# pvachon/tsl-sdr

Hardware: AMD Instinct MI355X
Metric: input IQ MSamp/s x channels demodulated (higher is better)
Workload: dtype int16

## Files before the change

tsl-sdr_amd/csrc/mfm_kernel.h:

```cpp
#pragma once

#include <stdint.h>

#define MFM_WAVE 64
#define MFM_CG 8
#define MFM_TG 2
#define MFM_NW 8
#define MFM_NT (MFM_NW * MFM_WAVE)

struct mfm_chan_info {
    uint64_t rot_base;
    uint32_t mu;
    uint32_t lam;
    uint32_t lam_magic;
    uint32_t pad0;
    uint32_t out_row;
    uint32_t rot_class;
};

#define MFM_RC_GENERAL 0u
#define MFM_RC_QUARTER 1u
#define MFM_RC_FLIP 2u
#define MFM_RC_IDENT 3u

// ... 127 lines not shown
    uint32_t stream_taps;
    uint32_t row_bytes;
    uint32_t split_rows;
    uint32_t kq_used;
    uint32_t nh;
    uint32_t kperm[4];
    uint32_t ng;
    uint32_t rb;
    uint32_t nstage_p;
    uint32_t shift;
    uint32_t tp_off;
    uint32_t *tail_dst;
    unsigned long long *cyc;
    unsigned long long *cyc_clear;
    uint32_t cyc_tag, pad2;
    const uint32_t *afrag;
    const int32_t *krow;
    const struct mfm_chan_info *info;
    const void *rot;
    const float2 *lut;
    int16_t *pcm;
    uint32_t *iq_dbg;
    const uint32_t *head;
    uint32_t head_n, pad3;
};
```

tsl-sdr_amd/csrc/mfm_kernel_v3.hip:

```cpp
#include <hip/hip_runtime.h>

#include <type_traits>

#include "mfm_kernel.h"
#include "mfm_numerics.h"

#include "mfm_v3_device.h"

#define MFM3_MF(d, a, b, c) "v_mfma_i32_16x16x64_i8 %[" #d "], %[" #a "], %[" #b "], " c "\n\t"
#define MFM3_RD(d, o) "ds_read_b128 %[" #d "], %[lb] offset:%[" #o "]\n\t"
#define MFM3_LA(d, a, b) "v_lshl_add_u32 %[" #d "], %[" #a "], 8, %[" #b "]\n\t"
#define MFM3_SH0(d, a) "v_lshrrev_b32_sdwa %[" #d "], 14, %[" #a "] dst_sel:WORD_0 dst_unused:UNUSED_PAD src0_sel:DWORD src1_sel:DWORD\n\t"
#define MFM3_SH1(d, a) "v_lshrrev_b32_sdwa %[" #d "], 14, %[" #a "] dst_sel:WORD_1 dst_unused:UNUSED_PRESERVE src0_sel:DWORD src1_sel:DWORD\n\t"

template <bool HAS_PREV, bool HAS_NEXT, int LO, int O2, int O3, int N0, int N1, bool REUSE = false>
static __device__ __forceinline__ void mfm3_group_d96(uint32_t lb, uint32_t ka, const mfm_v4i &al0, const mfm_v4i &al1,
                                                      const mfm_v4i &al2, const mfm_v4i &al3, const mfm_v4i &ah1,
                                                      const mfm_v4i &ah2, mfm_v4i &b0h, mfm_v4i &b0l, mfm_v4i &b1h,
                                                      mfm_v4i &b1l, mfm_v4i &b2h, mfm_v4i &b2l, const mfm_v4i (&accP)[3],
                                                      mfm_v4i (&acc)[3], uint32_t (&tP)[4])
{
    mfm_v4i hh, md, ll;
    uint32_t t0 = 0, t1 = 0, t2 = 0, t3 = 0;
    if (HAS_PREV) {
// ... 260 lines not shown
    static constexpr bool padded = DFIX == 25;
    static constexpr uint32_t row_bytes = padded ? 64u : 2u * D;
    static constexpr bool chunk_rows = !padded && (2u * D) % 64u != 0u;
    static constexpr uint32_t rows = padded ? MFM_V3_LEAD + MFM_V3_OT + 5u
                                            : MFM_V3_LEAD + MFM_V3_OT + (64u * 4u - 1u) / (2u * D);
    static constexpr uint32_t cpo = D / 8u, per = 4u * cpo;
    static constexpr uint32_t nchunks16 = (rows * 2u * D + 15u) / 16u;
    static constexpr uint32_t pitch_a = (nchunks16 + per - 1u) / per + 1u, pitch_b = 16u + 1u + (cpo * 3u + 12u) / per + 1u;
    static constexpr uint32_t pitch = pitch_a > pitch_b ? pitch_a : pitch_b;
    static constexpr uint32_t plane_t = ((per + 3u) * pitch * 16u + 63u) & ~63u;
    static constexpr uint32_t rs = padded ? 96u : mfm3_row_stride(D), sp = MFM3_SP;
    static constexpr uint32_t plane_pitch = chunk_rows ? plane_t : 4u * sp, buf_pitch = 2u * plane_pitch;
    static constexpr uint32_t ofs(uint32_t g, uint32_t kq)
    {
        if (chunk_rows) {
            const uint32_t x = cpo * g + 4u * kq;
            return ((x % per) * pitch + 1u + x / per) * 16u;
        }
        const uint32_t c = (64u * kq) / row_bytes, w = (64u * kq) % row_bytes;
        return ((g + c) & 3u) * sp + (1u + ((g + c) >> 2)) * rs + w;
    }
};

template <int KQ, bool DBG_IQ, int NCH, int AHM, int DFIX, int IN8, uint32_t RC = MFM_RC_GENERAL>
__global__ __launch_bounds__(MFM3_NT, 4) void mfm_channel_kernel_v3(const mfm_launch_v3 L)
{
    extern __shared__ __attribute__((aligned(16))) uint8_t smem[];

    const uint32_t tid = threadIdx.x;
    const uint32_t lane = tid & 63u;
    const uint32_t wave = __builtin_amdgcn_readfirstlane(tid >> 6);
    const uint32_t kg = lane >> 4, n = lane & 15u;
    using G = mfm3_geo<DFIX>;
    constexpr bool PADDED = DFIX != 0 && G::padded;
    constexpr uint32_t NCHS = PADDED ? 4u : (uint32_t)NCH;
    const uint32_t D = DFIX ? (uint32_t)DFIX : L.decim, row_bytes = PADDED ? 64u : 2u * D;
    const uint32_t rs = DFIX ? G::rs : L.rs;
    const uint32_t sp_pitch = DFIX ? G::sp : L.sp_pitch;
    const uint32_t plane_pitch = DFIX ? G::plane_pitch : L.plane_pitch, buf_pitch = DFIX ? G::buf_pitch : L.buf_pitch;
    const bool chunk_rows = DFIX ? G::chunk_rows : L.layout == 1u;
    const uint32_t t_per = DFIX ? G::per : L.t_per, t_pitch = DFIX ? G::pitch : L.t_pitch;
    const uint32_t ah_mask = AHM >= 0 ? (uint32_t)AHM : (uint32_t)__builtin_amdgcn_readfirstlane(L.ah_mask);
    const uint32_t lut_addr = (uint32_t)(uintptr_t)(smem + L.lut_off) | (MFM3_LUT_MODE == 2 ? 1u : 0u);
    const bool pcm_sys = L.pcm_scope != 0u;

    static_assert(MFM3_NT == 512, "one table dword per thread");
    const uint32_t lut_v = reinterpret_cast<const uint32_t *>(L.lut)[tid];
#if !MFM3_PROLOGUE
    reinterpret_cast<uint32_t *>(smem + L.lut_off)[MFM3_LUT_SLOT(tid)] = lut_v;
#endif

    uint32_t *sta_s = reinterpret_cast<uint32_t *>(smem + L.sta_off);
    uint32_t *sta2_s = sta_s + NCHS * MFM3_NT + 768u;
    uint16_t *sta16_s = reinterpret_cast<uint16_t *>(sta_s);
    if constexpr (PADDED) {
        constexpr int C = IN8 ? 8 : 4;
        const int delta = ((int)L.hist - (int)(MFM_V3_LEAD * 25u)) & (C - 1);
#pragma unroll
        for (int k = 0; k < C; k++) {
            const int i = C * (int)tid + k - delta;
            uint32_t off = 64u;
            if (i >= 0 && i < (int)(G::rows * 25u)) {
                const uint32_t row = (uint32_t)i / 25u, col = ((uint32_t)i % 25u) * 2u;
                off = (row & 3u) * sp_pitch + (row >> 2) * rs + col;
            }
            sta16_s[tid * 8u + (uint32_t)k] = (uint16_t)off;
        }
    }
#pragma unroll
    for (int j = 0; j < NCH && !PADDED; j++) {
        const uint32_t p8 = (tid + (uint32_t)j * MFM3_NT) * (IN8 ? 16u : 8u);
        if (chunk_rows) {
            const uint32_t sc = p8 >> 4, r = sc % t_per, c = sc / t_per;
            sta_s[j * MFM3_NT + tid] = (r * t_pitch + c) * 16u + (p8 & 15u);
            sta2_s[j * MFM3_NT + tid] = (r < 3u && c >= 1u) ? ((r + t_per) * t_pitch + c - 1u) * 16u + (p8 & 15u) : 0xffffffffu;
        } else {
            const uint32_t row = p8 / row_bytes, colb = p8 % row_bytes;
            sta_s[j * MFM3_NT + tid] = (row & 3u) * sp_pitch + (row >> 2) * rs + colb;
        }
    }

    uint32_t ofs[4][KQ], ofs_w[KQ];
#pragma unroll
    for (int kq = 0; kq < KQ; kq++) {
        const uint32_t c = DFIX ? (64u * kq) / row_bytes : L.cross[kq], w = DFIX ? (64u * kq) % row_bytes : L.within[kq];
        static_assert(!PADDED || (KQ == 6 && NCH == 1), "decimation 25: six rows per window, one staging chunk per thread");
#pragma unroll
        for (int g = 0; g < 4; g++) {
            ofs[g][kq] = ((g + c) & 3u) * sp_pitch + (1u + ((g + c) >> 2)) * rs + w;
        }
        ofs_w[kq] = ((3u + c) & 3u) * sp_pitch + ((3u + c) >> 2) * rs + w;
        if (chunk_rows) {
            const uint32_t cpo = t_per >> 2;
#pragma unroll
            for (int g = 0; g < 4; g++) {
                const uint32_t x = cpo * (uint32_t)g + 4u * (uint32_t)kq;
                ofs[g][kq] = ((x % t_per) * t_pitch + 1u + x / t_per) * 16u;
            }
            const uint32_t xw = cpo * 3u + 4u * (uint32_t)kq;
            ofs_w[kq] = ((xw % t_per) * t_pitch + xw / t_per) * 16u;
        }
    }
    const uint32_t lb0 = chunk_rows ? 16u * n + 16u * t_pitch * kg : n * rs + 16u * kg;

    auto stage_index = [&](uint32_t tile, int j) -> int {
        const uint32_t q = tid + (uint32_t)j * MFM3_NT;
        int gs = (int)(tile * MFM_V3_OT * D + L.hist) - (int)(MFM_V3_LEAD * D) + (IN8 ? 8 : 4) * (int)(q < L.nstage4 ? q : 0u);
        if constexpr (PADDED) {
            gs -= ((int)L.hist - (int)(MFM_V3_LEAD * 25u)) & ((IN8 ? 8 : 4) - 1);
        }
        gs = gs < 0 ? 0 : gs;
        return gs > (int)L.x_last4 ? (int)L.x_last4 : gs;
    };
    auto stage_load = [&](uint32_t tile, int j) -> uint4 {
        const int gs = stage_index(tile, j);
#if MFM3_NONTEMPORAL & 1
        const mfm_v4i ld = __builtin_nontemporal_load(
            reinterpret_cast<const mfm_v4i *>(reinterpret_cast<const uint8_t *>(L.x) + ((uint32_t)gs << (IN8 ? 1 : 2))));
        return make_uint4((uint32_t)ld[0], (uint32_t)ld[1], (uint32_t)ld[2], (uint32_t)ld[3]);
#else
        return *reinterpret_cast<const uint4 *>(reinterpret_cast<const uint8_t *>(L.x) + ((uint32_t)gs << (IN8 ? 1 : 2)));
#endif
    };
    auto stage_store = [&](uint32_t buf, int j, const uint4 &v) {
        if constexpr (PADDED) {
            if (tid < L.nstage4) {
                const uint4 o = *reinterpret_cast<const uint4 *>(sta16_s + tid * 8u);
                uint8_t *img = smem + buf * buf_pitch;
                const uint32_t vv[4] = { v.x, v.y, v.z, v.w }, oo[4] = { o.x, o.y, o.z, o.w };
                if (IN8) {
                    const uint32_t m = L.in8_xor;
#pragma unroll
                    for (int k = 0; k < 4; k++) {
                        const uint32_t w = vv[k] ^ m;
                        *reinterpret_cast<uint16_t *>(img + (oo[k] & 0xffffu)) = (uint16_t)w;
                        *reinterpret_cast<uint16_t *>(img + (oo[k] >> 16)) = (uint16_t)(w >> 16);
                    }
                } else {
#pragma unroll
                    for (int k = 0; k < 4; k++) {
                        const uint32_t off = (k & 1) ? oo[k >> 1] >> 16 : oo[k >> 1] & 0xffffu;
                        const uint32_t hi = __builtin_amdgcn_perm(vv[k], vv[k], 0x0c0c0301u);
                        const uint32_t lo = __builtin_amdgcn_perm(vv[k], vv[k], 0x0c0c0200u) ^ 0x8080u;
                        *reinterpret_cast<uint16_t *>(img + off) = (uint16_t)hi;
                        *reinterpret_cast<uint16_t *>(img + off + plane_pitch) = (uint16_t)lo;
                    }
                }
            }
            (void)j;
            return;
        }
        if (IN8) {
            if (tid + (uint32_t)j * MFM3_NT < L.nstage4) {
                const uint32_t m = L.in8_xor;
                const uint4 w = make_uint4(v.x ^ m, v.y ^ m, v.z ^ m, v.w ^ m);
                *reinterpret_cast<uint4 *>(smem + buf * buf_pitch + sta_s[j * MFM3_NT + tid]) = w;
                if (chunk_rows) {
                    const uint32_t a2 = sta2_s[j * MFM3_NT + tid];
                    if (a2 != 0xffffffffu) {
                        *reinterpret_cast<uint4 *>(smem + buf * buf_pitch + a2) = w;
                    }
                }
            }
        } else if (tid + (uint32_t)j * MFM3_NT < L.nstage4) {
            uint2 hi, lo;
            hi.x = __builtin_amdgcn_perm(v.y, v.x, 0x07050301u);
            hi.y = __builtin_amdgcn_perm(v.w, v.z, 0x07050301u);
            lo.x = __builtin_amdgcn_perm(v.y, v.x, 0x06040200u) ^ 0x80808080u;
            lo.y = __builtin_amdgcn_perm(v.w, v.z, 0x06040200u) ^ 0x80808080u;
            uint8_t *base = smem + buf * buf_pitch + sta_s[j * MFM3_NT + tid];
            *reinterpret_cast<uint2 *>(base) = hi;
            *reinterpret_cast<uint2 *>(base + plane_pitch) = lo;
            if (chunk_rows) {
                const uint32_t a2 = sta2_s[j * MFM3_NT + tid];
                if (a2 != 0xffffffffu) {
                    uint8_t *b2 = smem + buf * buf_pitch + a2;
                    *reinterpret_cast<uint2 *>(b2) = hi;
                    *reinterpret_cast<uint2 *>(b2 + plane_pitch) = lo;
                }
            }
        }
    };

    if (blockIdx.x == 0) {
        for (uint32_t i = tid; i < L.tail_n; i += MFM3_NT) {
            if (IN8) {
                reinterpret_cast<uint16_t *>(L.tail_dst)[i] = reinterpret_cast<const uint16_t *>(L.x)[L.tail_src + i];
            } else {
                L.tail_dst[i] = L.x[L.tail_src + i];
            }
        }
    }

    uint32_t item = blockIdx.x, chunk, slice;
    if (!mfm3_decode_item(L, item, &chunk, &slice)) {
        return;
    }
    const uint32_t stamp_t0 = mfm3_stamp_lo(L.cyc ? __builtin_amdgcn_s_memtime() : 0ull), stamp_r0 = mfm3_stamp_lo(L.cyc ? __builtin_amdgcn_s_memrealtime() : 0ull);
    uint32_t tile = (uint32_t)(((uint64_t)chunk * L.ntiles) / L.nchunks);
    uint32_t tend = (uint32_t)(((uint64_t)(chunk + 1u) * L.ntiles) / L.nchunks);
    mfm_v4i a_h[KQ], a_l[KQ];
    mfm_v4i *krow_s = reinterpret_cast<mfm_v4i *>(smem + L.sta_off + NCHS * MFM3_NT * 4u) + wave * 4u + kg;
    uint32_t slice_loaded = 0xffffffffu;
    {
        uint4 v[NCH];
#pragma unroll
        for (int j = 0; j < NCH; j++) {
            v[j] = stage_load(tile, j);
        }
#if MFM3_PROLOGUE
        const uint32_t rb0 = slice * 8u + wave;
        mfm_v4i krow0 = { 0, 0, 0, 0 };
        if (rb0 < L.nrb) {
            const mfm_v4i *ap = reinterpret_cast<const mfm_v4i *>(L.afrag) + (size_t)rb0 * KQ * 2 * 64 + mfm3_opaque(lane);
#pragma unroll
            for (int kq = 0; kq < KQ; kq++) {
                a_h[kq] = ap[(kq * 2 + 0) * 64];
                a_l[kq] = ap[(kq * 2 + 1) * 64];
            }
            krow0 = *reinterpret_cast<const mfm_v4i *>(L.krow + (size_t)rb0 * 16 + 4 * mfm3_opaque(kg));
        }
        reinterpret_cast<uint32_t *>(smem + L.lut_off)[MFM3_LUT_SLOT(tid)] = lut_v;
#endif
        if constexpr (IN8 == 0) {
            if (L.head_n != 0u && tile == 0u) {
#pragma unroll
                for (int j = 0; j < NCH; j++) {
                    const uint32_t gs = (uint32_t)stage_index(0u, j);
                    uint32_t w[4] = { v[j].x, v[j].y, v[j].z, v[j].w };
#pragma unroll
                    for (int k = 0; k < 4; k++) {
                        if (gs + (uint32_t)k < L.head_n) {
                            w[k] = L.head[gs + (uint32_t)k];
                        }
                    }
                    v[j] = make_uint4(w[0], w[1], w[2], w[3]);
                }
            }
        }
#pragma unroll
        for (int j = 0; j < NCH; j++) {
            stage_store(0, j, v[j]);
        }
#if MFM3_PROLOGUE
        if (rb0 < L.nrb) {
            asm volatile("s_waitcnt vmcnt(0)" ::: "memory");
            if (n == 0) {
                *krow_s = krow0;
            }
#pragma unroll
            for (int kq = 0; kq < KQ; kq++) {
                asm volatile("" : "+v"(a_h[kq]), "+v"(a_l[kq]));
            }
            slice_loaded = slice;
        }
#endif
    }
    __syncthreads();

    const int prio_matrix = wave >= 4 ? 1 : 0;
    uint2 *fold_s = reinterpret_cast<uint2 *>(smem + L.sta_off + NCHS * MFM3_NT * 4u + 512u) + (wave * 4u + kg) * 2u;
    uint32_t *xq_s = reinterpret_cast<uint32_t *>(smem + L.sta_off + NCHS * MFM3_NT * 4u + 1024u) + (wave * 4u + kg) * 16u;
    uint32_t cur = 0;
    bool first_of_chunk = true;

    uint32_t kb8[2] = { 0, 0 };
    uint32_t voff[2] = { 0, 0 };
    uint32_t hist[2] = { 0, 0 };
    bool ch_ok[2] = { false, false };
    bool w_exact = false;

    auto advance = [&](uint32_t &it, uint32_t &ch, uint32_t &sl, uint32_t &ti, uint32_t &te, bool &first) -> bool {
        ti += 1u;
        first = false;
        if (ti >= te) {
            it += gridDim.x;
            const bool v = mfm3_decode_item(L, it, &ch, &sl);
            ti = (uint32_t)(((uint64_t)ch * L.ntiles) / L.nchunks);
            te = (uint32_t)(((uint64_t)(ch + 1u) * L.ntiles) / L.nchunks);
            first = true;
            return v;
        }
        return true;
    };
    constexpr bool EARLY = IN8 != 0 || MFM3_EARLY16;
    uint4 pre[NCH];
    if (EARLY) {
        uint32_t a_item = item, a_chunk = chunk, a_slice = slice, a_tile = tile, a_tend = tend;
        bool a_first = false;
        const bool a_valid = advance(a_item, a_chunk, a_slice, a_tile, a_tend, a_first);
#pragma unroll
        for (int j = 0; j < NCH; j++) {
            pre[j] = stage_load(a_valid ? a_tile : tile, j);
        }
    }

    while (true) {
        uint32_t n_item = item, n_chunk = chunk, n_slice = slice, n_tile = tile, n_tend = tend;
        bool n_first = false;
        const bool n_valid = advance(n_item, n_chunk, n_slice, n_tile, n_tend, n_first);
        if (!EARLY) {
#pragma unroll
            for (int j = 0; j < NCH; j++) {
                pre[j] = stage_load(n_valid ? n_tile : tile, j);
            }
            __builtin_amdgcn_sched_barrier(MFM3_SCHED_ALL_BUT_VMEM);
        }

        if (prio_matrix) {
            __builtin_amdgcn_s_setprio(1);
        } else {
            __builtin_amdgcn_s_setprio(0);
        }
        const uint32_t rb = slice * 8u + wave;
        const bool rb_valid = rb < L.nrb;
        const uint32_t lb = lb0 + cur * buf_pitch;
        const uint8_t *img = smem;
        const uint32_t first_out = tile * MFM_V3_OT;

        uint32_t f[4][2];
        uint4 rva[2][MFM3_ROT4 ? 1 : 2];
        if (rb_valid) {
            const uint32_t ch0 = rb * 8u + 2u * kg;
            if (slice != slice_loaded) {
                const mfm_v4i *ap = reinterpret_cast<const mfm_v4i *>(L.afrag) + (size_t)rb * KQ * 2 * 64 + mfm3_opaque(lane);
#pragma unroll
                for (int kq = 0; kq < KQ; kq++) {
                    a_h[kq] = ap[(kq * 2 + 0) * 64];
                    a_l[kq] = ap[(kq * 2 + 1) * 64];
                }
                const mfm_v4i krow = *reinterpret_cast<const mfm_v4i *>(L.krow + (size_t)rb * 16 + 4 * mfm3_opaque(kg));
                asm volatile("s_waitcnt vmcnt(0)" ::: "memory");
                if (n == 0) {
                    *krow_s = krow;
                }
#pragma unroll
                for (int kq = 0; kq < KQ; kq++) {
                    asm volatile("" : "+v"(a_h[kq]), "+v"(a_l[kq]));
                }
// ... 110 lines not shown
#else
                        const uint2 e = reinterpret_cast<const uint2 *>(L.rot)[inf.x + kw];
                        wrx[c] = e.x;
                        wry[c] = e.y;
#endif
                    }
                }
                if constexpr (RC == MFM_RC_GENERAL) {
                    w_exact = MFM3_WAVE_EXACT &&
                              __builtin_amdgcn_ballot_w64(cls[0] == MFM_RC_GENERAL || cls[1] == MFM_RC_GENERAL) == 0;
#pragma unroll
                    for (int c = 0; c < 2; c++) {
                        kb8[c] = w_exact ? 0u : kbg[c];
                        if (n == 0) {
                            fold_s[c] = fog[c];
                        }
                    }
                } else if constexpr (RC == MFM_RC_FLIP) {
                    kb8[0] = sgn[0];
                    kb8[1] = sgn[1];
                }
                if ((RC == MFM_RC_GENERAL && w_exact) || RC == MFM_RC_QUARTER) {
                    if (n < 4u) {
#pragma unroll
                        for (int c = 0; c < 2; c++) {
                            xq_s[c * 8 + n] = selq[c];
                            xq_s[c * 8 + 4 + n] = sgq[c];
                        }
                    }
                }
                if (first_out != 0 || L.hist != 0) {
                    uint32_t fw[2], qw[2];
                    uint32_t ow[KQ];
#pragma unroll
                    for (int kq = 0; kq < KQ; kq++) {
                        ow[kq] = ofs_w[kq];
                    }
                    column_group(ow, fw);
                    derotate2(fw, wrx, wry, qw);
                    hist[0] = qw[0];
                    hist[1] = qw[1];
                }
            }

            if constexpr (DFIX != 0 && KQ == 4 && AHM == 0x6 && IN8 == 0) {
#define MFM3_OFS(g, kq) ((int)G::ofs((g), (kq)))
                constexpr int LO = (int)G::plane_pitch;
                const uint32_t ka = (uint32_t)(uintptr_t)krow_s;
                mfm_v4i ph, pl, qh, ql, rh = { 0, 0, 0, 0 }, rl = { 0, 0, 0, 0 };
                asm volatile("ds_read_b128 %[x0h], %[lb] offset:%[a]\n\t"
// ... 21 lines not shown
                    f[1][0] = t[0];
                    f[1][1] = t[2];
                    mfm3_group_d96<true, false, LO, MFM3_OFS(3, 2), MFM3_OFS(3, 3), 0, 0>(
                        lb, ka, a_l[0], a_l[1], a_l[2], a_l[3], a_h[1], a_h[2], ph, pl, rh, rl, qh, ql, acc0, acc1, t);
                    f[2][0] = t[0];
                    f[2][1] = t[2];
                } else {
                    mfm3_group_d96<false, true, LO, MFM3_OFS(0, 2), MFM3_OFS(0, 3), MFM3_OFS(1, 0), MFM3_OFS(1, 1)>(
                        lb, ka, a_l[0], a_l[1], a_l[2], a_l[3], a_h[1], a_h[2], ph, pl, qh, ql, rh, rl, none, acc0, t);
                    mfm3_group_d96<true, true, LO, MFM3_OFS(1, 2), MFM3_OFS(1, 3), MFM3_OFS(2, 0), MFM3_OFS(2, 1)>(
                        lb, ka, a_l[0], a_l[1], a_l[2], a_l[3], a_h[1], a_h[2], qh, ql, rh, rl, ph, pl, acc0, acc1, t);
                    f[0][0] = t[0];
                    f[0][1] = t[2];
                    mfm3_group_d96<true, true, LO, MFM3_OFS(2, 2), MFM3_OFS(2, 3), MFM3_OFS(3, 0), MFM3_OFS(3, 1)>(
                        lb, ka, a_l[0], a_l[1], a_l[2], a_l[3], a_h[1], a_h[2], rh, rl, ph, pl, qh, ql, acc1, acc0, t);
                    f[1][0] = t[0];
                    f[1][1] = t[2];
                    mfm3_group_d96<true, false, LO, MFM3_OFS(3, 2), MFM3_OFS(3, 3), 0, 0>(
                        lb, ka, a_l[0], a_l[1], a_l[2], a_l[3], a_h[1], a_h[2], ph, pl, qh, ql, rh, rl, acc0, acc1, t);
                    f[2][0] = t[0];
                    f[2][1] = t[2];
                }
                __builtin_amdgcn_sched_barrier(0);
                if constexpr (RC == MFM_RC_GENERAL) {
#pragma unroll
                    for (int c = 0; c < 2; c++) {
                        const uint8_t *rp = reinterpret_cast<const uint8_t *>(L.rot) + kb8[c];
                        rva[c][0] = *reinterpret_cast<const uint4 *>(rp);
#if !MFM3_ROT4
                        rva[c][1] = *reinterpret_cast<const uint4 *>(rp + 16);
#endif
                    }
                }
                __builtin_amdgcn_sched_barrier(0);
                settle();
                finish(acc1, f[3]);
#undef MFM3_OFS
            } else if constexpr (DFIX != 0 && KQ == 4 && AHM == 0x6 && IN8 != 0) {
#define MFM3_OFS(g, kq) ((int)G::ofs((g), (kq)))
                const uint32_t ka = (uint32_t)(uintptr_t)krow_s;
                mfm_v4i pb, qb, rb2 = { 0, 0, 0, 0 };
                asm volatile("ds_read_b128 %[x0], %[lb] offset:%[a]\n\t"
                             "ds_read_b128 %[x1], %[lb] offset:%[b]\n\t"
                             : [x0] "=&v"(pb), [x1] "=&v"(qb)
                             : [lb] "v"(lb), [a] "n"(MFM3_OFS(0, 0)), [b] "n"(MFM3_OFS(0, 1))
                             : "memory");
                mfm_v4i acc0[3], acc1[3];
// ... 5 lines not shown
                    mfm3_group_d96_b8<false, true, IN8, MFM3_OFS(0, 2), MFM3_OFS(0, 3), MFM3_OFS(1, 0), MFM3_OFS(1, 1), true>(
                        lb, ka, a_l[0], a_l[1], a_l[2], a_l[3], a_h[1], a_h[2], pb, qb, rb2, none, acc0, t);
                    mfm3_group_d96_b8<true, true, IN8, MFM3_OFS(1, 2), MFM3_OFS(1, 3), MFM3_OFS(2, 0), MFM3_OFS(2, 1), true>(
                        lb, ka, a_l[0], a_l[1], a_l[2], a_l[3], a_h[1], a_h[2], pb, rb2, qb, acc0, acc1, t);
                    f[0][0] = t[0];
                    f[0][1] = t[2];
                    mfm3_group_d96_b8<true, true, IN8, MFM3_OFS(2, 2), MFM3_OFS(2, 3), MFM3_OFS(3, 0), MFM3_OFS(3, 1), true>(
                        lb, ka, a_l[0], a_l[1], a_l[2], a_l[3], a_h[1], a_h[2], pb, qb, rb2, acc1, acc0, t);
                    f[1][0] = t[0];
                    f[1][1] = t[2];
                } else {
                    mfm3_group_d96_b8<false, true, IN8, MFM3_OFS(0, 2), MFM3_OFS(0, 3), MFM3_OFS(1, 0), MFM3_OFS(1, 1)>(
                        lb, ka, a_l[0], a_l[1], a_l[2], a_l[3], a_h[1], a_h[2], pb, qb, rb2, none, acc0, t);
                    mfm3_group_d96_b8<true, true, IN8, MFM3_OFS(1, 2), MFM3_OFS(1, 3), MFM3_OFS(2, 0), MFM3_OFS(2, 1)>(
                        lb, ka, a_l[0], a_l[1], a_l[2], a_l[3], a_h[1], a_h[2], qb, rb2, pb, acc0, acc1, t);
                    f[0][0] = t[0];
                    f[0][1] = t[2];
                    mfm3_group_d96_b8<true, true, IN8, MFM3_OFS(2, 2), MFM3_OFS(2, 3), MFM3_OFS(3, 0), MFM3_OFS(3, 1)>(
                        lb, ka, a_l[0], a_l[1], a_l[2], a_l[3], a_h[1], a_h[2], rb2, pb, qb, acc1, acc0, t);
                    f[1][0] = t[0];
                    f[1][1] = t[2];
                }
                __builtin_amdgcn_sched_barrier(0);
                if constexpr (RC == MFM_RC_GENERAL) {
#pragma unroll
                    for (int c = 0; c < 2; c++) {
                        const uint8_t *rp = reinterpret_cast<const uint8_t *>(L.rot) + kb8[c];
                        rva[c][0] = *reinterpret_cast<const uint4 *>(rp);
#if !MFM3_ROT4
                        rva[c][1] = *reinterpret_cast<const uint4 *>(rp + 16);
#endif
                    }
                }
                __builtin_amdgcn_sched_barrier(0);
                if constexpr (TOEP) {
                    mfm3_group_d96_b8<true, false, IN8, MFM3_OFS(3, 2), MFM3_OFS(3, 3), 0, 0>(
                        lb, ka, a_l[0], a_l[1], a_l[2], a_l[3], a_h[1], a_h[2], pb, rb2, qb, acc0, acc1, t);
                } else {
                    mfm3_group_d96_b8<true, false, IN8, MFM3_OFS(3, 2), MFM3_OFS(3, 3), 0, 0>(
                        lb, ka, a_l[0], a_l[1], a_l[2], a_l[3], a_h[1], a_h[2], pb, qb, rb2, acc0, acc1, t);
                }
                f[2][0] = t[0];
                f[2][1] = t[2];
                settle();
                finish(acc1, f[3]);
#undef MFM3_OFS
            } else {
#pragma unroll
            for (int g = 0; g < 4; g++) {
                uint32_t og[KQ];
#pragma unroll
                for (int kq = 0; kq < KQ; kq++) {
                    og[kq] = ofs[g][kq];
                }
                column_group(og, f[g]);
                if (g == 1) {
                    __builtin_amdgcn_sched_barrier(0);
                    if constexpr (RC == MFM_RC_GENERAL) {
#pragma unroll
                        for (int c = 0; c < 2; c++) {
                            const uint8_t *rp = reinterpret_cast<const uint8_t *>(L.rot) + kb8[c];
                            rva[c][0] = *reinterpret_cast<const uint4 *>(rp);
#if !MFM3_ROT4
                            rva[c][1] = *reinterpret_cast<const uint4 *>(rp + 16);
#endif
                        }
                    }
                    __builtin_amdgcn_sched_barrier(0);
                }
            }
            }
        }

#pragma unroll
        for (int j = 0; j < NCH; j++) {
            stage_store(cur ^ 1u, j, pre[j]);
        }
#if !MFM3_BARRIER_LATE
        __syncthreads();
#endif
        __builtin_amdgcn_s_setprio(2);
        if (EARLY) {
            uint32_t a_item = n_item, a_chunk = n_chunk, a_slice = n_slice, a_tile = n_tile, a_tend = n_tend;
            bool a_first = false;
            const bool a_valid = n_valid && advance(a_item, a_chunk, a_slice, a_tile, a_tend, a_first);
#pragma unroll
            for (int j = 0; j < NCH; j++) {
                pre[j] = stage_load(a_valid ? a_tile : tile, j);
            }
            __builtin_amdgcn_sched_barrier(MFM3_SCHED_ALL_BUT_VMEM);
        }
        if (rb_valid) {
            const uint32_t n_left = L.n_new - first_out;
            uint32_t q[4][2];
#pragma unroll
            for (int c = 0; c < 2; c++) {
                if ((RC == MFM_RC_GENERAL && w_exact) || RC == MFM_RC_QUARTER) {
                    const uint4 sel4 = *reinterpret_cast<const uint4 *>(xq_s + c * 8);
                    const uint4 sg4 = *reinterpret_cast<const uint4 *>(xq_s + c * 8 + 4);
                    const uint32_t sel[4] = { sel4.x, sel4.y, sel4.z, sel4.w }, sg[4] = { sg4.x, sg4.y, sg4.z, sg4.w };
#pragma unroll
                    for (int g = 0; g < 4; g++) {
                        const uint32_t t = __builtin_amdgcn_perm(f[g][c], f[g][c], sel[g]);
                        asm("v_pk_mul_lo_u16 %0, %1, %2" : "=v"(q[g][c]) : "v"(t), "v"(sg[g]));
                    }
                } else if constexpr (RC == MFM_RC_GENERAL) {
#pragma unroll
                    for (int h = 0; h < 2; h++) {
#if MFM3_ROT4
                        const uint32_t r0 = h ? rva[c][0].z : rva[c][0].x, r1 = h ? rva[c][0].w : rva[c][0].y;
                        const uint32_t fin[2] = { f[2 * h][c], f[2 * h + 1][c] };
// ... 46 lines not shown
                    }
                } else {
#pragma unroll
                    for (int g = 0; g < 4; g++) {
                        if (ch_ok[c] && 4u * n + (uint32_t)g < n_left) {
                            *reinterpret_cast<int16_t *>(reinterpret_cast<uint8_t *>(L.pcm) + voff[c] + 2u * g) = (int16_t)pcm[g];
                            if (DBG_IQ) {
                                *reinterpret_cast<uint32_t *>(reinterpret_cast<uint8_t *>(L.iq_dbg) + 2u * (size_t)voff[c] + 4u * g) = q[g][c];
                            }
                        }
                    }
                }
#if MFM3_EPI_SERIAL
                if (c == 0) {
                    __builtin_amdgcn_sched_barrier(0);
                }
#endif
            }
#pragma unroll
            for (int c = 0; c < 2; c++) {
                if (RC == MFM_RC_GENERAL && !w_exact) {
                    const uint2 fo = fold_s[c];
                    kb8[c] += MFM_V3_OT * MFM3_ES;
                    kb8[c] = kb8[c] >= fo.x + 4u * MFM3_ES * n ? kb8[c] - fo.y : kb8[c];
                }
                voff[c] += MFM_V3_OT * 2u;
            }
        }

#if MFM3_BARRIER_LATE
        __syncthreads();
#endif
        if (!n_valid) {
            break;
        }
        cur ^= 1u;
        item = n_item;
        chunk = n_chunk;
        slice = n_slice;
        tile = n_tile;
        tend = n_tend;
        first_of_chunk = n_first;
    }
    mfm3_stamp_end(L, stamp_t0, stamp_r0);
}

__global__ __launch_bounds__(MFM3_NT) void mfm3_disc_test_kernel(const int *s_re, const int *s_im, int *pcm, uint32_t n4, const float2 *lut)
{
    __shared__ __attribute__((aligned(16))) uint32_t tbl[512];
    tbl[MFM3_LUT_SLOT(threadIdx.x)] = reinterpret_cast<const uint32_t *>(lut)[threadIdx.x];
    __syncthreads();
    const uint32_t t = blockIdx.x * MFM3_NT + threadIdx.x;
    if (t >= n4) {
        return;
    }
    int re[4], im[4], out[4];
#pragma unroll
    for (int i = 0; i < 4; i++) {
        re[i] = s_re[4 * t + i];
        im[i] = s_im[4 * t + i];
    }
    mfm3_discriminate4(re, im, (uint32_t)(uintptr_t)tbl, out);
#pragma unroll
    for (int i = 0; i < 4; i++) {
        pcm[4 * t + i] = out[i];
    }
}
// ... 71 lines not shown
        default: MFM3_LAUNCH(KQ_, DBG_, 8, AHM_); break;                                                     \
        }                                                                                                    \
    } while (0)
#define MFM3_LAUNCH_D(KQ_, AHM_)                                                                             \
    do {                                                                                                     \
        if (dbg_iq) {                                                                                        \
            MFM3_LAUNCH_N(KQ_, true, -1);                                                                    \
        } else {                                                                                             \
            MFM3_LAUNCH_N(KQ_, false, AHM_);                                                                 \
        }                                                                                                    \
    } while (0)
#define MFM3_LAUNCH_8(KQ_, IN8_)                                                                             \
    do {                                                                                                     \
        switch (nch) {                                                                                       \
        case 1: MFM3_LAUNCH_F(KQ_, false, 1, -1, 0, IN8_); break;                                            \
        case 2: MFM3_LAUNCH_F(KQ_, false, 2, -1, 0, IN8_); break;                                            \
        case 3: MFM3_LAUNCH_F(KQ_, false, 3, -1, 0, IN8_); break;                                            \
        default: MFM3_LAUNCH_F(KQ_, false, 4, -1, 0, IN8_); break;                                           \
        }                                                                                                    \
    } while (0)
#define MFM3_LAUNCH_8K(IN8_)                                                                                 \
    do {                                                                                                     \
        if (L->decim == 96 && L->kq == 4 && nch == 2 && L->ah_mask == 0x6u && L->rs == mfm3_row_stride(96) &&      \
            L->sp_pitch == MFM3_SP) {                                                                        \
            MFM3_LAUNCH_RC(4, 2, 0x6, 96, IN8_);                                                             \
        } else if (L->decim == 40 && L->kq == 4 && nch == 1 && L->ah_mask == 0x6u && geo40) {                \
            MFM3_LAUNCH_F(4, false, 1, 0x6, 40, IN8_);                                                       \
        } else {                                                                                             \
            switch (L->kq) {                                                                                 \
            case 1: MFM3_LAUNCH_8(1, IN8_); break;                                                           \
            case 2: MFM3_LAUNCH_8(2, IN8_); break;                                                           \
            case 4: MFM3_LAUNCH_8(4, IN8_); break;                                                           \
            default: return hipErrorInvalidValue;                                                            \
            }                                                                                                \
        }                                                                                                    \
    } while (0)
    const bool geo40 = L->layout == 1u && L->t_per == mfm3_geo<40>::per && L->t_pitch == mfm3_geo<40>::pitch &&
                       L->plane_pitch == mfm3_geo<40>::plane_pitch && L->buf_pitch == mfm3_geo<40>::buf_pitch;
    if (L->layout == 2u) {
        if (L->decim != 25u || L->kq != 6u || L->rs != mfm3_geo<25>::rs || L->sp_pitch != mfm3_geo<25>::sp || (dbg_iq && L->in8 != 0u)) {
            return hipErrorInvalidValue;
        }
        if (dbg_iq) {
            if ((L->ah_mask & ~0xeu) == 0u) {
                *kfn_out = reinterpret_cast<const void *>(&mfm_channel_kernel_v3<6, true, 1, 0xe, 25, 0>);
            } else {
                *kfn_out = reinterpret_cast<const void *>(&mfm_channel_kernel_v3<6, true, 1, -1, 25, 0>);
            }
            return hipSuccess;
// ... 13 lines not shown
        } else if (L->in8 == 14u) {
            MFM3_LAUNCH_25(14);
        } else if (L->in8 == 0u) {
            MFM3_LAUNCH_25(0);
        } else {
            return hipErrorInvalidValue;
        }
#undef MFM3_LAUNCH_25
        return hipSuccess;
    }
    if (L->in8) {
        if (dbg_iq || nch > 4 || (L->in8 != 7u && L->in8 != 14u)) {
            return hipErrorInvalidValue;
        }
        if (L->in8 == 7u) {
            MFM3_LAUNCH_8K(7);
        } else {
            MFM3_LAUNCH_8K(14);
        }
        return hipSuccess;
    }
#ifndef MFM3_NO_FIX
    if (L->decim == 96 && L->kq == 4 && nch == 4 && !dbg_iq && L->ah_mask == 0x6u && L->rs == mfm3_row_stride(96) &&
        L->sp_pitch == MFM3_SP) {
        MFM3_LAUNCH_RC(4, 4, 0x6, 96, 0);
        return hipSuccess;
    }
    if (L->decim == 40 && L->kq == 4 && nch == 2 && !dbg_iq && L->ah_mask == 0x6u && geo40) {
        MFM3_LAUNCH_F(4, false, 2, 0x6, 40, 0);
        return hipSuccess;
    }
#endif
    switch (L->kq) {
    case 1: MFM3_LAUNCH_D(1, -1); break;
    case 2: MFM3_LAUNCH_D(2, -1); break;
    case 4:
        if (L->ah_mask == 0x6u) {
            MFM3_LAUNCH_D(4, 0x6);
        } else {
            MFM3_LAUNCH_D(4, -1);
        }
        break;
    default: return hipErrorInvalidValue;
    }
#undef MFM3_LAUNCH_D
#undef MFM3_LAUNCH_8K
#undef MFM3_LAUNCH_8
#undef MFM3_LAUNCH_N
#undef MFM3_LAUNCH_RC
#undef MFM3_LAUNCH_F
#undef MFM3_LAUNCH
// ... 23 lines not shown
```

tsl-sdr_amd/csrc/mfm_plan.hip:

```cpp
#include <algorithm>
#include <cstdarg>
#include <cstdio>
#include <cstring>
#include <map>

#include "mfm_plan.h"
#include "mfm_numerics.h"

extern "C" hipError_t mfm_select_channel_kernel(int opl, int dbg_iq, const void **kfn_out);
extern "C" hipError_t mfm_select_channel_kernel_mfma(const mfm_launch_mfma *L, int dbg_iq, const void **kfn_out,
                                                     uint32_t *waves_per_simd_out);
extern "C" hipError_t mfm_select_channel_kernel_v3(const mfm_launch_v3 *L, int dbg_iq, const void **kfn_out);
extern "C" uint32_t mfm_rot_entry_bytes_v3(void);
extern "C" uint32_t mfm_sp_pitch_v3(void);
extern "C" uint32_t mfm_v3l_wg_per_cu(const mfm_launch_v3 *L);
extern "C" __attribute__((visibility("hidden"))) void mfm_internal_set_error(const char *msg);

namespace {

constexpr uint32_t kMaxOutputsPerTile = 128;
constexpr uint32_t kSlice128MinChannels = 512;
constexpr uint32_t kPcmWriteThroughMinChannels = 512;
constexpr uint64_t kMaxRotEntries = 1ull << 26;

// ... 423 lines not shown
        p.v_rc = MFM_RC_GENERAL;
    }
}

void fill_v3(const KernelPlan &p, uint32_t flags, int fmt, mfm_launch_v3 &V)
{
    V.decim = p.D;
    V.x_last4 = p.v_shift ? p.cap_in - 1u : (p.cap_in - 4u) & ~3u;
    V.kq = p.m_ks;
    V.rs = p.v_rs;
    V.sp_pitch = p.v_sp_pitch;
    V.plane_pitch = 4u * p.v_sp_pitch;
    V.buf_pitch = 8u * p.v_sp_pitch;
    V.nstage4 = p.v_nstage4;
    V.lut_off = 16u * p.v_sp_pitch;
    V.sta_off = V.lut_off + 2048u;
    for (int k = 0; k < 4; k++) {
        V.cross[k] = p.v_cross[k];
        V.within[k] = p.v_within[k];
    }
    V.layout = p.v_layout;
    V.t_per = p.v_t_per;
    V.t_pitch = p.v_t_pitch;
    if (3u == p.v_layout) {
        V.plane_pitch = p.v_plane;
        V.buf_pitch = 2u * p.v_plane;
        V.lut_off = 4u * p.v_plane;
        V.sta_off = V.lut_off + 2048u;
        V.tp_off = V.sta_off + p.v_sta_bytes;
        V.row_bytes = p.m_row_bytes;
        V.split_rows = (p.D % 4u) != 0u ? 1u : 0u;
        V.kq = p.v_kq;
        V.kq_used = p.m_kq_used;
        V.nh = p.v_nh;
        for (int k = 0; k < 4; k++) {
            V.kperm[k] = p.v_kperm[k];
        }
        V.ng = p.v_ng;
        V.rb = p.v_rb;
        V.nstage_p = p.v_nstage_p;
        V.shift = p.v_shift;
        if (p.v_shift) {
            V.sp_pitch = p.v_copy_pitch;
        }
    }
    V.nslices = p.v_nslices;
// ... 372 lines not shown
```

tsl-sdr_amd/csrc/mfm_v3_device.h:

```cpp
#pragma once

typedef int mfm_v4i __attribute__((ext_vector_type(4)));

#define MFM3_NT 512u
#ifndef MFM3_EARLY16
#define MFM3_EARLY16 1
#endif
#ifndef MFM3_WAVE_EXACT
#define MFM3_WAVE_EXACT 1
#endif
#ifndef MFM3_PROLOGUE
#define MFM3_PROLOGUE 1
#endif
#ifndef MFM3_BARRIER_LATE
#define MFM3_BARRIER_LATE 0
#endif
#ifndef MFM3_ROT4
#define MFM3_ROT4 1
#endif
#define MFM3_ES (MFM3_ROT4 ? 4u : 8u)
#ifndef MFM3_NONTEMPORAL
#define MFM3_NONTEMPORAL 2
#endif
#ifndef MFM3_SP
#define MFM3_SP 4096u
#endif
#ifndef MFM3_EPI_SERIAL
#define MFM3_EPI_SERIAL 0
#endif
#ifndef MFM3_DIV_STEPS
#define MFM3_DIV_STEPS 1
#endif
#ifndef MFM3_TOEPLITZ
#define MFM3_TOEPLITZ 1
#endif
#ifndef MFM3_LUT_MODE
#define MFM3_LUT_MODE 1
#endif
#define MFM3_LUT_SLOT(t) (MFM3_LUT_MODE == 1 ? (t) : ((t) >> 1) + (((t)&1u) << 8))
#define MFM3_SCHED_ALL_BUT_VMEM 0x38F

static __device__ __forceinline__ uint32_t mfm3_combine(int hh, int md, int ll)
{
    uint32_t t, a;
    asm("v_lshl_add_u32 %0, %1, 8, %2" : "=v"(t) : "v"(hh), "v"(md));
    asm("v_lshl_add_u32 %0, %1, 8, %2" : "=v"(a) : "v"(t), "v"(ll));
    return a;
}

static __device__ __forceinline__ void mfm3_round_pack2(const uint32_t re_b[2], const uint32_t im_b[2], uint32_t p[2])
{
    uint32_t p0, p1;
    asm("v_lshrrev_b32_sdwa %0, 14, %2 dst_sel:WORD_0 dst_unused:UNUSED_PAD src0_sel:DWORD src1_sel:DWORD\n\t"
        "v_lshrrev_b32_sdwa %1, 14, %3 dst_sel:WORD_0 dst_unused:UNUSED_PAD src0_sel:DWORD src1_sel:DWORD\n\t"
        "v_lshrrev_b32_sdwa %0, 14, %4 dst_sel:WORD_1 dst_unused:UNUSED_PRESERVE src0_sel:DWORD src1_sel:DWORD\n\t"
        "v_lshrrev_b32_sdwa %1, 14, %5 dst_sel:WORD_1 dst_unused:UNUSED_PRESERVE src0_sel:DWORD src1_sel:DWORD\n\t"
        "s_nop 0"
// ... 259 lines not shown
}

static __device__ __forceinline__ uint32_t mfm3_stamp_lo(uint64_t t)
{
    uint32_t lo = (uint32_t)t;
    asm volatile("" : "+s"(lo));
    return lo;
}

static __device__ __forceinline__ void mfm3_stamp_end(const mfm_launch_v3 &L, uint32_t t0, uint32_t r0)
{
    if (L.cyc != nullptr && threadIdx.x == 0) {
        const uint64_t tag = (uint64_t)(L.cyc_tag & 0xffffffu) << 40;
        const uint64_t dt = (uint32_t)((uint32_t)__builtin_amdgcn_s_memtime() - t0), dr = (uint32_t)((uint32_t)__builtin_amdgcn_s_memrealtime() - r0);
        atomicMax(L.cyc, (unsigned long long)(tag | dt));
        atomicMax(L.cyc + 1, (unsigned long long)(tag | dr));
        if (blockIdx.x == 0) {
            L.cyc_clear[0] = 0ull;
            L.cyc_clear[1] = 0ull;
        }
    }
}

static __device__ __forceinline__ bool mfm3_decode_item(const mfm_launch_v3 &L, uint32_t item, uint32_t *chunk, uint32_t *slice)
{
    const uint32_t xcd = item & 7u, seq = item >> 3;
    *chunk = (seq / L.nslices) * 8u + xcd;
    *slice = seq % L.nslices;
    return item < L.nitems && *chunk < L.nchunks;
}
```

Measured before the change: 37.99 million.

## Reorder staging loads lead-last, trim redundant staging chunks, skip rotation on exact windows

Staging of input samples is reordered so that, for consecutive tiles in a chunk, only the new body samples are loaded and the lead overlap is reused. Per-thread staging chunks beyond the needed count are skipped via a compile-time full-chunk count plus a per-wave ownership test. Rotation table reads are skipped when the window is exact. Several values are rematerialized through opaque asm (lane base, shared pointers, nslices/nchunks) to cut register pressure. This adds an extra lead_chunks launch field and a host-side geometry check to guard the fixed-decimation fast paths.

```diff
diff --git a/tsl-sdr_amd/csrc/mfm_kernel.h b/tsl-sdr_amd/csrc/mfm_kernel.h
--- a/tsl-sdr_amd/csrc/mfm_kernel.h
+++ b/tsl-sdr_amd/csrc/mfm_kernel.h
@@ -173,5 +173,6 @@
     int16_t *pcm;
     uint32_t *iq_dbg;
     const uint32_t *head;
-    uint32_t head_n, pad3;
+    uint32_t head_n;
+    uint32_t lead_chunks;
 };
diff --git a/tsl-sdr_amd/csrc/mfm_kernel_v3.hip b/tsl-sdr_amd/csrc/mfm_kernel_v3.hip
--- a/tsl-sdr_amd/csrc/mfm_kernel_v3.hip
+++ b/tsl-sdr_amd/csrc/mfm_kernel_v3.hip
@@ -306,6 +306,14 @@
     }
 };
 
+template <int DFIX>
+static bool mfm3_geo_counts(const mfm_launch_v3 *L)
+{
+    using G = mfm3_geo<DFIX>;
+    const uint32_t per = L->in8 ? 8u : 4u;
+    return L->nstage4 == G::rows * G::D / 4u / (per / 4u) && L->lead_chunks == MFM_V3_LEAD * G::D / per;
+}
+
 template <int KQ, bool DBG_IQ, int NCH, int AHM, int DFIX, int IN8, uint32_t RC = MFM_RC_GENERAL>
 __global__ __launch_bounds__(MFM3_NT, 4) void mfm_channel_kernel_v3(const mfm_launch_v3 L)
 {
@@ -351,9 +359,18 @@
             sta16_s[tid * 8u + (uint32_t)k] = (uint16_t)off;
         }
     }
+    constexpr bool LEADF = MFM3_LEAD_FIRST != 0 && DFIX != 0 && !PADDED;
+    constexpr bool TRIMF = MFM3_STAGE_TRIM != 0 && DFIX != 0 && !PADDED;
+    constexpr int NFULL = !TRIMF ? NCH : (int)(((G::rows - (LEADF ? MFM_V3_LEAD : 0u)) * G::D / (IN8 ? 8u : 4u)) / MFM3_NT);
+    static_assert(NFULL <= NCH, "a thread's staging chunks");
+    auto stage_order = [](int i) -> int { return i < NCH - NFULL ? NFULL + i : i - (NCH - NFULL); };
+    const uint32_t lead_q = LEADF ? L.lead_chunks : 0u;
+    const uint32_t nbody = L.nstage4 - lead_q;
 #pragma unroll
     for (int j = 0; j < NCH && !PADDED; j++) {
-        const uint32_t p8 = (tid + (uint32_t)j * MFM3_NT) * (IN8 ? 16u : 8u);
+        const uint32_t q = tid + (uint32_t)j * MFM3_NT;
+        const uint32_t qi = LEADF ? (q < nbody ? q + lead_q : q - nbody) : q;
+        const uint32_t p8 = qi * (IN8 ? 16u : 8u);
         if (chunk_rows) {
             const uint32_t sc = p8 >> 4, r = sc % t_per, c = sc / t_per;
             sta_s[j * MFM3_NT + tid] = (r * t_pitch + c) * 16u + (p8 & 15u);
@@ -385,19 +402,41 @@
             ofs_w[kq] = ((xw % t_per) * t_pitch + xw / t_per) * 16u;
         }
     }
-    const uint32_t lb0 = chunk_rows ? 16u * n + 16u * t_pitch * kg : n * rs + 16u * kg;
-
-    auto stage_index = [&](uint32_t tile, int j) -> int {
-        const uint32_t q = tid + (uint32_t)j * MFM3_NT;
-        int gs = (int)(tile * MFM_V3_OT * D + L.hist) - (int)(MFM_V3_LEAD * D) + (IN8 ? 8 : 4) * (int)(q < L.nstage4 ? q : 0u);
+    auto lane_base = [&]() -> uint32_t {
+        const uint32_t t = mfm3_opaque(tid), tn = t & 15u, tkg = (t >> 4) & 3u;
+        return chunk_rows ? 16u * tn + 16u * t_pitch * tkg : tn * rs + 16u * tkg;
+    };
+
+    auto stage_count = [&](bool first) -> uint32_t { return first ? L.nstage4 : nbody; };
+    auto stage_owns = [&](int j, uint32_t cnt) -> bool {
+        return j < NFULL || wave * 64u + (uint32_t)j * MFM3_NT < cnt;
+    };
+    auto stage_index = [&](uint32_t tile, int j, bool first) -> int {
+        int gs;
+        if constexpr (LEADF) {
+            const int base = (int)(tile * MFM_V3_OT * D + L.hist) - (int)(MFM_V3_LEAD * D);
+            if (first && (!TRIMF || j >= NFULL)) {
+                const uint32_t q = mfm3_opaque(tid) + (uint32_t)j * MFM3_NT;
+                const uint32_t qi = q < nbody ? q + lead_q : q < L.nstage4 ? q - nbody : 0u;
+                gs = base + (IN8 ? 8 : 4) * (int)qi;
+            } else if (TRIMF) {
+                gs = base + (IN8 ? 8 : 4) * (int)(lead_q + (uint32_t)j * MFM3_NT) + (IN8 ? 8 : 4) * (int)tid;
+            } else {
+                const uint32_t q = tid + (uint32_t)j * MFM3_NT;
+                gs = base + (IN8 ? 8 : 4) * (int)(q < nbody ? q + lead_q : lead_q);
+            }
+        } else {
+            const uint32_t q = tid + (uint32_t)j * MFM3_NT;
+            gs = (int)(tile * MFM_V3_OT * D + L.hist) - (int)(MFM_V3_LEAD * D) + (IN8 ? 8 : 4) * (int)(q < L.nstage4 ? q : 0u);
+        }
         if constexpr (PADDED) {
             gs -= ((int)L.hist - (int)(MFM_V3_LEAD * 25u)) & ((IN8 ? 8 : 4) - 1);
         }
         gs = gs < 0 ? 0 : gs;
         return gs > (int)L.x_last4 ? (int)L.x_last4 : gs;
     };
-    auto stage_load = [&](uint32_t tile, int j) -> uint4 {
-        const int gs = stage_index(tile, j);
+    auto stage_load = [&](uint32_t tile, int j, bool first) -> uint4 {
+        const int gs = stage_index(tile, j, first);
 #if MFM3_NONTEMPORAL & 1
         const mfm_v4i ld = __builtin_nontemporal_load(
             reinterpret_cast<const mfm_v4i *>(reinterpret_cast<const uint8_t *>(L.x) + ((uint32_t)gs << (IN8 ? 1 : 2))));
@@ -406,7 +445,7 @@
         return *reinterpret_cast<const uint4 *>(reinterpret_cast<const uint8_t *>(L.x) + ((uint32_t)gs << (IN8 ? 1 : 2)));
 #endif
     };
-    auto stage_store = [&](uint32_t buf, int j, const uint4 &v) {
+    auto stage_store = [&](uint32_t buf, int j, const uint4 &v, uint32_t cnt) {
         if constexpr (PADDED) {
             if (tid < L.nstage4) {
                 const uint4 o = *reinterpret_cast<const uint4 *>(sta16_s + tid * 8u);
@@ -431,11 +470,13 @@
                     }
                 }
             }
-            (void)j;
+            (void)j, (void)cnt;
             return;
         }
+        int lim = (int)cnt - j * (int)MFM3_NT;
+        asm volatile("" : "+s"(lim));
         if (IN8) {
-            if (tid + (uint32_t)j * MFM3_NT < L.nstage4) {
+            if ((int)tid < lim) {
                 const uint32_t m = L.in8_xor;
                 const uint4 w = make_uint4(v.x ^ m, v.y ^ m, v.z ^ m, v.w ^ m);
                 *reinterpret_cast<uint4 *>(smem + buf * buf_pitch + sta_s[j * MFM3_NT + tid]) = w;
@@ -446,7 +487,7 @@
                     }
                 }
             }
-        } else if (tid + (uint32_t)j * MFM3_NT < L.nstage4) {
+        } else if ((int)tid < lim) {
             uint2 hi, lo;
             hi.x = __builtin_amdgcn_perm(v.y, v.x, 0x07050301u);
             hi.y = __builtin_amdgcn_perm(v.w, v.z, 0x07050301u);
@@ -477,20 +518,30 @@
     }
 
     uint32_t item = blockIdx.x, chunk, slice;
-    if (!mfm3_decode_item(L, item, &chunk, &slice)) {
+    if (!mfm3_decode_item<true>(L, item, &chunk, &slice)) {
         return;
     }
     const uint32_t stamp_t0 = mfm3_stamp_lo(L.cyc ? __builtin_amdgcn_s_memtime() : 0ull), stamp_r0 = mfm3_stamp_lo(L.cyc ? __builtin_amdgcn_s_memrealtime() : 0ull);
-    uint32_t tile = (uint32_t)(((uint64_t)chunk * L.ntiles) / L.nchunks);
-    uint32_t tend = (uint32_t)(((uint64_t)(chunk + 1u) * L.ntiles) / L.nchunks);
+    auto chunk_start = [&](uint32_t ch) -> uint32_t {
+        uint32_t nc = L.nchunks;
+        asm volatile("" : "+s"(nc));
+        return (uint32_t)(((uint64_t)ch * L.ntiles) / nc);
+    };
+    uint32_t tile = chunk_start(chunk);
+    uint32_t tend = chunk_start(chunk + 1u);
     mfm_v4i a_h[KQ], a_l[KQ];
-    mfm_v4i *krow_s = reinterpret_cast<mfm_v4i *>(smem + L.sta_off + NCHS * MFM3_NT * 4u) + wave * 4u + kg;
+    auto wkg16 = [&]() -> uint32_t { return mfm3_opaque(tid) & ~15u; };
+#define krow_s (reinterpret_cast<mfm_v4i *>(smem + L.sta_off + NCHS * MFM3_NT * 4u + wkg16()))
     uint32_t slice_loaded = 0xffffffffu;
     {
         uint4 v[NCH];
-#pragma unroll
-        for (int j = 0; j < NCH; j++) {
-            v[j] = stage_load(tile, j);
+        const uint32_t cnt0 = stage_count(true);
+#pragma unroll
+        for (int i = 0; i < NCH; i++) {
+            const int j = stage_order(i);
+            if (stage_owns(j, cnt0)) {
+                v[j] = stage_load(tile, j, true);
+            }
         }
 #if MFM3_PROLOGUE
         const uint32_t rb0 = slice * 8u + wave;
@@ -510,7 +561,10 @@
             if (L.head_n != 0u && tile == 0u) {
 #pragma unroll
                 for (int j = 0; j < NCH; j++) {
-                    const uint32_t gs = (uint32_t)stage_index(0u, j);
+                    if (!stage_owns(j, cnt0)) {
+                        continue;
+                    }
+                    const uint32_t gs = (uint32_t)stage_index(0u, j, true);
                     uint32_t w[4] = { v[j].x, v[j].y, v[j].z, v[j].w };
 #pragma unroll
                     for (int k = 0; k < 4; k++) {
@@ -524,7 +578,9 @@
         }
 #pragma unroll
         for (int j = 0; j < NCH; j++) {
-            stage_store(0, j, v[j]);
+            if (stage_owns(j, cnt0)) {
+                stage_store(0, j, v[j], cnt0);
+            }
         }
 #if MFM3_PROLOGUE
         if (rb0 < L.nrb) {
@@ -543,8 +599,8 @@
     __syncthreads();
 
     const int prio_matrix = wave >= 4 ? 1 : 0;
-    uint2 *fold_s = reinterpret_cast<uint2 *>(smem + L.sta_off + NCHS * MFM3_NT * 4u + 512u) + (wave * 4u + kg) * 2u;
-    uint32_t *xq_s = reinterpret_cast<uint32_t *>(smem + L.sta_off + NCHS * MFM3_NT * 4u + 1024u) + (wave * 4u + kg) * 16u;
+#define fold_s (reinterpret_cast<uint2 *>(smem + L.sta_off + NCHS * MFM3_NT * 4u + 512u + wkg16()))
+#define xq_s (reinterpret_cast<uint32_t *>(smem + L.sta_off + NCHS * MFM3_NT * 4u + 1024u + 4u * wkg16()))
     uint32_t cur = 0;
     bool first_of_chunk = true;
 
@@ -559,9 +615,9 @@
         first = false;
         if (ti >= te) {
             it += gridDim.x;
-            const bool v = mfm3_decode_item(L, it, &ch, &sl);
-            ti = (uint32_t)(((uint64_t)ch * L.ntiles) / L.nchunks);
-            te = (uint32_t)(((uint64_t)(ch + 1u) * L.ntiles) / L.nchunks);
+            const bool v = mfm3_decode_item<true>(L, it, &ch, &sl);
+            ti = chunk_start(ch);
+            te = chunk_start(ch + 1u);
             first = true;
             return v;
         }
@@ -569,13 +625,18 @@
     };
     constexpr bool EARLY = IN8 != 0 || MFM3_EARLY16;
     uint4 pre[NCH];
+    uint32_t pre_cnt = nbody;
     if (EARLY) {
         uint32_t a_item = item, a_chunk = chunk, a_slice = slice, a_tile = tile, a_tend = tend;
         bool a_first = false;
         const bool a_valid = advance(a_item, a_chunk, a_slice, a_tile, a_tend, a_first);
-#pragma unroll
-        for (int j = 0; j < NCH; j++) {
-            pre[j] = stage_load(a_valid ? a_tile : tile, j);
+        pre_cnt = stage_count(a_valid && a_first);
+#pragma unroll
+        for (int i = 0; i < NCH; i++) {
+            const int j = stage_order(i);
+            if (stage_owns(j, pre_cnt)) {
+                pre[j] = stage_load(a_valid ? a_tile : tile, j, a_valid && a_first);
+            }
         }
     }
 
@@ -584,9 +645,13 @@
         bool n_first = false;
         const bool n_valid = advance(n_item, n_chunk, n_slice, n_tile, n_tend, n_first);
         if (!EARLY) {
-#pragma unroll
-            for (int j = 0; j < NCH; j++) {
-                pre[j] = stage_load(n_valid ? n_tile : tile, j);
+            pre_cnt = stage_count(n_valid && n_first);
+#pragma unroll
+            for (int i = 0; i < NCH; i++) {
+                const int j = stage_order(i);
+                if (stage_owns(j, pre_cnt)) {
+                    pre[j] = stage_load(n_valid ? n_tile : tile, j, n_valid && n_first);
+                }
             }
             __builtin_amdgcn_sched_barrier(MFM3_SCHED_ALL_BUT_VMEM);
         }
@@ -598,7 +663,7 @@
         }
         const uint32_t rb = slice * 8u + wave;
         const bool rb_valid = rb < L.nrb;
-        const uint32_t lb = lb0 + cur * buf_pitch;
+        const uint32_t lb = lane_base() + cur * buf_pitch;
         const uint8_t *img = smem;
         const uint32_t first_out = tile * MFM_V3_OT;
 
@@ -755,10 +820,11 @@
                 }
                 if ((RC == MFM_RC_GENERAL && w_exact) || RC == MFM_RC_QUARTER) {
                     if (n < 4u) {
+                        uint32_t *xq_n = xq_s + (mfm3_opaque(tid) & 3u);
 #pragma unroll
                         for (int c = 0; c < 2; c++) {
-                            xq_s[c * 8 + n] = selq[c];
-                            xq_s[c * 8 + 4 + n] = sgq[c];
+                            xq_n[c * 8] = selq[c];
+                            xq_n[c * 8 + 4] = sgq[c];
                         }
                     }
                 }
@@ -826,7 +892,7 @@
                     f[2][1] = t[2];
                 }
                 __builtin_amdgcn_sched_barrier(0);
-                if constexpr (RC == MFM_RC_GENERAL) {
+                if (RC == MFM_RC_GENERAL && !(MFM3_EXACT_NO_ROT && w_exact)) {
 #pragma unroll
                     for (int c = 0; c < 2; c++) {
                         const uint8_t *rp = reinterpret_cast<const uint8_t *>(L.rot) + kb8[c];
@@ -878,7 +944,7 @@
                     f[1][1] = t[2];
                 }
                 __builtin_amdgcn_sched_barrier(0);
-                if constexpr (RC == MFM_RC_GENERAL) {
+                if (RC == MFM_RC_GENERAL && !(MFM3_EXACT_NO_ROT && w_exact)) {
 #pragma unroll
                     for (int c = 0; c < 2; c++) {
                         const uint8_t *rp = reinterpret_cast<const uint8_t *>(L.rot) + kb8[c];
@@ -912,7 +978,7 @@
                 column_group(og, f[g]);
                 if (g == 1) {
                     __builtin_amdgcn_sched_barrier(0);
-                    if constexpr (RC == MFM_RC_GENERAL) {
+                    if (RC == MFM_RC_GENERAL && !(MFM3_EXACT_NO_ROT && w_exact)) {
 #pragma unroll
                         for (int c = 0; c < 2; c++) {
                             const uint8_t *rp = reinterpret_cast<const uint8_t *>(L.rot) + kb8[c];
@@ -930,7 +996,9 @@
 
 #pragma unroll
         for (int j = 0; j < NCH; j++) {
-            stage_store(cur ^ 1u, j, pre[j]);
+            if (stage_owns(j, pre_cnt)) {
+                stage_store(cur ^ 1u, j, pre[j], pre_cnt);
+            }
         }
 #if !MFM3_BARRIER_LATE
         __syncthreads();
@@ -940,9 +1008,13 @@
             uint32_t a_item = n_item, a_chunk = n_chunk, a_slice = n_slice, a_tile = n_tile, a_tend = n_tend;
             bool a_first = false;
             const bool a_valid = n_valid && advance(a_item, a_chunk, a_slice, a_tile, a_tend, a_first);
-#pragma unroll
-            for (int j = 0; j < NCH; j++) {
-                pre[j] = stage_load(a_valid ? a_tile : tile, j);
+            pre_cnt = stage_count(a_valid && a_first);
+#pragma unroll
+            for (int i = 0; i < NCH; i++) {
+                const int j = stage_order(i);
+                if (stage_owns(j, pre_cnt)) {
+                    pre[j] = stage_load(a_valid ? a_tile : tile, j, a_valid && a_first);
+                }
             }
             __builtin_amdgcn_sched_barrier(MFM3_SCHED_ALL_BUT_VMEM);
         }
@@ -1035,7 +1107,7 @@
                 if (RC == MFM_RC_GENERAL && !w_exact) {
                     const uint2 fo = fold_s[c];
                     kb8[c] += MFM_V3_OT * MFM3_ES;
-                    kb8[c] = kb8[c] >= fo.x + 4u * MFM3_ES * n ? kb8[c] - fo.y : kb8[c];
+                    kb8[c] = kb8[c] >= fo.x + 4u * MFM3_ES * (mfm3_opaque(tid) & 15u) ? kb8[c] - fo.y : kb8[c];
                 }
                 voff[c] += MFM_V3_OT * 2u;
             }
@@ -1056,6 +1128,9 @@
         first_of_chunk = n_first;
     }
     mfm3_stamp_end(L, stamp_t0, stamp_r0);
+#undef krow_s
+#undef fold_s
+#undef xq_s
 }
 
 __global__ __launch_bounds__(MFM3_NT) void mfm3_disc_test_kernel(const int *s_re, const int *s_im, int *pcm, uint32_t n4, const float2 *lut)
@@ -1173,9 +1248,9 @@
 #define MFM3_LAUNCH_8K(IN8_)                                                                                 \
     do {                                                                                                     \
         if (L->decim == 96 && L->kq == 4 && nch == 2 && L->ah_mask == 0x6u && L->rs == mfm3_row_stride(96) &&      \
-            L->sp_pitch == MFM3_SP) {                                                                        \
+            L->sp_pitch == MFM3_SP && mfm3_geo_counts<96>(L)) {                                              \
             MFM3_LAUNCH_RC(4, 2, 0x6, 96, IN8_);                                                             \
-        } else if (L->decim == 40 && L->kq == 4 && nch == 1 && L->ah_mask == 0x6u && geo40) {                \
+        } else if (L->decim == 40 && L->kq == 4 && nch == 1 && L->ah_mask == 0x6u && geo40 && mfm3_geo_counts<40>(L)) { \
             MFM3_LAUNCH_F(4, false, 1, 0x6, 40, IN8_);                                                       \
         } else {                                                                                             \
             switch (L->kq) {                                                                                 \
@@ -1235,11 +1310,11 @@
     }
 #ifndef MFM3_NO_FIX
     if (L->decim == 96 && L->kq == 4 && nch == 4 && !dbg_iq && L->ah_mask == 0x6u && L->rs == mfm3_row_stride(96) &&
-        L->sp_pitch == MFM3_SP) {
+        L->sp_pitch == MFM3_SP && mfm3_geo_counts<96>(L)) {
         MFM3_LAUNCH_RC(4, 4, 0x6, 96, 0);
         return hipSuccess;
     }
-    if (L->decim == 40 && L->kq == 4 && nch == 2 && !dbg_iq && L->ah_mask == 0x6u && geo40) {
+    if (L->decim == 40 && L->kq == 4 && nch == 2 && !dbg_iq && L->ah_mask == 0x6u && geo40 && mfm3_geo_counts<40>(L)) {
         MFM3_LAUNCH_F(4, false, 2, 0x6, 40, 0);
         return hipSuccess;
     }
diff --git a/tsl-sdr_amd/csrc/mfm_plan.hip b/tsl-sdr_amd/csrc/mfm_plan.hip
--- a/tsl-sdr_amd/csrc/mfm_plan.hip
+++ b/tsl-sdr_amd/csrc/mfm_plan.hip
@@ -469,6 +469,7 @@
     V.layout = p.v_layout;
     V.t_per = p.v_t_per;
     V.t_pitch = p.v_t_pitch;
+    V.lead_chunks = p.v_layout <= 1u ? MFM_V3_LEAD * p.D / (fmt != MFM_IN_CS16 ? 8u : 4u) : 0u;
     if (3u == p.v_layout) {
         V.plane_pitch = p.v_plane;
         V.buf_pitch = 2u * p.v_plane;
diff --git a/tsl-sdr_amd/csrc/mfm_v3_device.h b/tsl-sdr_amd/csrc/mfm_v3_device.h
--- a/tsl-sdr_amd/csrc/mfm_v3_device.h
+++ b/tsl-sdr_amd/csrc/mfm_v3_device.h
@@ -33,6 +33,15 @@
 #endif
 #ifndef MFM3_TOEPLITZ
 #define MFM3_TOEPLITZ 1
+#endif
+#ifndef MFM3_LEAD_FIRST
+#define MFM3_LEAD_FIRST 1
+#endif
+#ifndef MFM3_STAGE_TRIM
+#define MFM3_STAGE_TRIM 1
+#endif
+#ifndef MFM3_EXACT_NO_ROT
+#define MFM3_EXACT_NO_ROT 1
 #endif
 #ifndef MFM3_LUT_MODE
 #define MFM3_LUT_MODE 1
@@ -338,10 +347,15 @@
     }
 }
 
+template <bool REMAT = false>
 static __device__ __forceinline__ bool mfm3_decode_item(const mfm_launch_v3 &L, uint32_t item, uint32_t *chunk, uint32_t *slice)
 {
     const uint32_t xcd = item & 7u, seq = item >> 3;
-    *chunk = (seq / L.nslices) * 8u + xcd;
-    *slice = seq % L.nslices;
+    uint32_t ns = L.nslices;
+    if (REMAT) {
+        asm volatile("" : "+s"(ns));
+    }
+    *chunk = (seq / ns) * 8u + xcd;
+    *slice = seq % ns;
     return item < L.nitems && *chunk < L.nchunks;
 }
```

Result: no change. 37.80 million (-0.5%).
